# JuanTarrio/rebvo

Hardware: NVIDIA H100
Metric: frames/sec @752x480 EuRoC replay (synthetic stand-in), detect+track+map; pose ATE vs reference in `parity` (higher is better)
Workload: dtype f32 scale space/detector + f64 tracker/EKF

## Files before the change

rebvo_b200/csrc/capi.cu:

```cuda
#include <math.h>
#include <stdlib.h>
#include <new>

#include "common.cuh"
#include "tracker.cuh"

int rb_detect_upload_pinv(rb_ctx *c, const double *tab);

static void box_plan_one(double sigma, int box_n, int *box_d, double *sigma_r) {
    const double wideal = sqrt(12 * sigma * sigma / box_n + 1);
    int wl = (int)wideal;
    const int tmp = wl / 2;
    if (tmp * 2 == wl) wl--;
    const int m = (int)round((3 * box_n + 4 * box_n * wl + box_n * wl * wl - 12 * sigma * sigma) / (4 + 4 * wl));
    int i = 0;
    for (; i < m && i < box_n; i++) box_d[i] = wl;
    for (; i < box_n; i++) box_d[i] = wl + 2;
    *sigma_r = sqrt((m * wl * wl + (box_n - m) * (wl + 2.0) * (wl + 2.0) - box_n) / 12.0);
}

static void plane_fit_pinv(int ws, double *out) {
    const int n = (2 * ws + 1) * (2 * ws + 1);
    double Phi[(2 * RB_PLANE_FIT_MAX + 1) * (2 * RB_PLANE_FIT_MAX + 1)][3];
    int k = 0;
// ... 28 lines not shown
    for (int r = 0; r < 3; r++)
        for (k = 0; k < n; k++) {
            double s = 0;
            for (int c = 0; c < 3; c++) s += B[r][c] * Phi[k][c];
            out[r * n + k] = s;
        }
}

static const double *plane_fit_tables() {
    static double tab[RB_PINV_DOUBLES];
    static std::once_flag once;
    std::call_once(once, [] {
        for (int r = 1; r <= RB_PLANE_FIT_MAX; r++) plane_fit_pinv(r, tab + rb_pinv_offset(r));
    });
    return tab;
}

__device__ __forceinline__ void pack_one(const KLSoA &kl, int i, rb_keyline *dst) {
    rb_keyline k;
    k.p_inx = kl.p_inx[i];
    float2 v = kl.m_m[i];
    k.m_m[0] = v.x; k.m_m[1] = v.y;
    v = kl.u_m[i];
    k.u_m[0] = v.x; k.u_m[1] = v.y;
    k.n_m = kl.n_m[i];
    k.score = 0.f;
    v = kl.c_p[i];
    k.c_p[0] = v.x; k.c_p[1] = v.y;
    k._pad0 = 0;
    k.rho = kl.rho[i];
    k.s_rho = kl.s_rho[i];
    k.rho_nr = RB_RHO_INIT;
    k.s_rho_nr = RB_RHO_MAX;
    k.rho0 = kl.rho0[i];
    k.s_rho0 = kl.s_rho0[i];
    v = kl.p_m[i];
    k.p_m[0] = v.x; k.p_m[1] = v.y;
    v = kl.p_m_0[i];
    k.p_m_0[0] = v.x; k.p_m_0[1] = v.y;
    k.m_id = kl.m_id[i];
    k.m_id_f = kl.m_id_f[i];
    k.m_id_kf = -1;
    k.m_num = kl.m_num[i];
    v = kl.m_m0[i];
    k.m_m0[0] = v.x; k.m_m0[1] = v.y;
    k.n_m0 = kl.n_m0[i];
    k.p_id = kl.p_id[i];
    k.n_id = kl.n_id[i];
    k.net_id = -1;
    k.stereo_m_id = -1;
    k.stereo_rho = RB_RHO_INIT;
    k.stereo_s_rho = RB_RHO_MAX;
    *dst = k;
}
__global__ void k_pack_aos(KLSoA kl, const MapState *st, rb_keyline *out) {
    const int i = blockIdx.x * blockDim.x + threadIdx.x;
    if (i >= st->kn) return;
    pack_one(kl, i, out + i);
}

__global__ void __launch_bounds__(128) k_pack_aos_ind(KLSoA kl, const MapState *st, unsigned char *const *base, size_t offset) {
    __shared__ __align__(16) rb_keyline rec[128];
    const int kn = st->kn;
    const int i0 = blockIdx.x * 128;
    if (i0 >= kn) return;
    const int i = i0 + threadIdx.x;
    if (i < kn) pack_one(kl, i, &rec[threadIdx.x]);
    __syncthreads();
    const int nrec = kn - i0 < 128 ? kn - i0 : 128;
    const int n8 = nrec * (int)(sizeof(rb_keyline) / 8);
    uint2 *dst = reinterpret_cast<uint2 *>(*base + offset) + (size_t)i0 * (sizeof(rb_keyline) / 8);
    const uint2 *src = reinterpret_cast<const uint2 *>(rec);
    for (int k = threadIdx.x; k < n8; k += 128) dst[k] = src[k];
}
int rb_map_pack_aos_enqueue(rb_ctx *c, rb_map *m, unsigned char *const *base, size_t offset) {
    k_pack_aos_ind<<<rb_div_up(c->kcap, 128), 128, 0, c->stream>>>(m->kl, m->st, base, offset);
    RB_LAUNCH_CHECK();
    return RB_OK;
}

__global__ void k_unpack_aos(KLSoA kl, MapState *st, const rb_keyline *in, int kn) {
    const int i = blockIdx.x * blockDim.x + threadIdx.x;
    if (i == 0) st->kn = kn;
    if (i >= kn) return;
    const rb_keyline k = in[i];
    kl.p_inx[i] = k.p_inx;
    kl.m_m[i] = make_float2(k.m_m[0], k.m_m[1]);
    kl.u_m[i] = make_float2(k.u_m[0], k.u_m[1]);
    kl.n_m[i] = k.n_m;
    kl.c_p[i] = make_float2(k.c_p[0], k.c_p[1]);
    kl.rho[i] = k.rho;
    kl.s_rho[i] = k.s_rho;
    kl.rho0[i] = k.rho0;
    kl.s_rho0[i] = k.s_rho0;
    kl.p_m[i] = make_float2(k.p_m[0], k.p_m[1]);
    kl.p_m_0[i] = make_float2(k.p_m_0[0], k.p_m_0[1]);
    kl.m_id[i] = k.m_id;
    kl.m_id_f[i] = k.m_id_f;
    kl.m_num[i] = k.m_num;
    kl.m_m0[i] = make_float2(k.m_m0[0], k.m_m0[1]);
    kl.n_m0[i] = k.n_m0;
    kl.p_id[i] = k.p_id;
    kl.n_id[i] = k.n_id;
    kl.pack[2 * i] = make_float4(k.m_m[0], k.m_m[1], k.c_p[0], k.c_p[1]);
    kl.pack[2 * i + 1] = make_float4(k.u_m[0], k.u_m[1], k.n_m, 0.f);
}

__global__ void k_fill_int(int *p, int v, size_t n) {
    size_t i = (size_t)blockIdx.x * blockDim.x + threadIdx.x;
    if (i < n) p[i] = v;
}

extern "C" int rb_ctx_create(rb_ctx **out, int device, const rb_camera *cam, double sigma0, double ksigma,
                             int kl_capacity) {
    if (!out || !cam) return RB_ERR_ARG;
    *out = nullptr;
    int ndev = 0;
    if (cudaGetDeviceCount(&ndev) != cudaSuccess || ndev <= 0 || device >= ndev) return RB_ERR_NO_DEVICE;
    if (cam->w % 4 || cam->w < 32 || cam->h < 32 || kl_capacity < 1) return RB_ERR_ARG;
    rb_ctx *c = new (std::nothrow) rb_ctx;
    if (!c) return RB_ERR_ARG;
    memset(c, 0, sizeof(*c));
    c->mtx = new (std::nothrow) std::recursive_mutex;
    if (!c->mtx) {
        delete c;
        return RB_ERR_ARG;
    }
    c->device = device;
    c->cam = *cam;
    c->w = cam->w;
    c->h = cam->h;
    c->N = cam->w * cam->h;
    c->ppx = cam->ppx;
    c->ppy = cam->ppy;
    c->zfm = (double)((cam->zfx + cam->zfy) / 2);
    c->sigma0 = sigma0;
    c->ksigma = ksigma;
    c->kcap = kl_capacity;
    {
        const char *ds = getenv("REBVO_B200_DOG_SUB");
        c->dog_sub = ds ? atoi(ds) : 0;
        if (c->dog_sub < 0) c->dog_sub = 0;
        const char *pd = getenv("REBVO_B200_PDL");
        c->pdl = !(pd && atoi(pd) == 0);
        const char *mp = getenv("REBVO_B200_MIN_PERSIST");
        c->min_persist = !(mp && atoi(mp) == 0);
        const char *mc = getenv("REBVO_B200_MIN_CLUSTER");
        c->min_cluster = !(mc && atoi(mc) == 0);
        const char *rs = getenv("REBVO_B200_ROWSCAN");
        c->rowscan_mode = rs ? atoi(rs) : 2;
        c->mu_xchg = !(getenv("REBVO_B200_MU_XCHG") && atoi(getenv("REBVO_B200_MU_XCHG")) == 0);
        c->row_ns = getenv("REBVO_B200_ROW_NS") ? atoi(getenv("REBVO_B200_ROW_NS")) : 0;
        c->colscan_mode = getenv("REBVO_B200_COLSCAN") ? atoi(getenv("REBVO_B200_COLSCAN")) : 0;
    }
    box_plan_one(sigma0, 3, c->plan.d[0], &c->plan.sigma_r[0]);
    box_plan_one(c->plan.sigma_r[0] * ksigma, 3, c->plan.d[1], &c->plan.sigma_r[1]);
    int r = RB_OK;
    auto fail = [&](int code) {
        *out = c;
        return code;
    };
#define CK(call)                                                                                  \
    do {                                                                                          \
        cudaError_t e__ = (call);                                                                 \
        if (e__ != cudaSuccess) {                                                                 \
            snprintf(c->err, sizeof(c->err), "%s:%d %s: %s", __FILE__, __LINE__, #call,           \
                     cudaGetErrorString(e__));                                                    \
            return fail(RB_ERR_CUDA);                                                             \
        }                                                                                         \
    } while (0)
    CK(cudaSetDevice(device));
    cudaDeviceProp prop;
    CK(cudaGetDeviceProperties(&prop, device));
    c->sm_count = prop.multiProcessorCount;
    rb_minimizer_cluster_setup(c);
    if ((r = rb_dog_device_setup(c))) return fail(r);
    {
        int lo = 0, hi = 0;
        cudaDeviceGetStreamPriorityRange(&lo, &hi);
        const char *pe = getenv("REBVO_B200_PRIO");
        CK(cudaStreamCreateWithPriority(&c->stream, cudaStreamNonBlocking, (pe && atoi(pe) == 0) ? lo : hi));
    }
    c->nseg = c->h * rb_div_up(c->w, 32);
    CK(cudaMalloc(&c->seg_cnt, sizeof(int) * c->nseg));
    CK(cudaMalloc(&c->cand, sizeof(float4) * (size_t)c->N));
    c->red_cap = 1024;
    CK(cudaMalloc(&c->red_part, sizeof(double) * 32 * c->red_cap));
    CK(cudaMalloc(&c->ticket, sizeof(unsigned int) * 16));
    CK(cudaMemset(c->ticket, 0, sizeof(unsigned int) * 16));
    CK(cudaMallocHost(&c->pinned, 1 << 16));
    CK(cudaMalloc(&c->dev_small, 1 << 16));
    CK(cudaMemset(c->dev_small, 0, 1 << 16));
    {
        const int mm_init[2] = {-1, 0x7f7fffff};
        CK(cudaMemcpy((char *)c->dev_small + RB_DS_REEST, mm_init, sizeof(mm_init), cudaMemcpyHostToDevice));
    }
    if ((r = rb_detect_upload_pinv(c, plane_fit_tables()))) return fail(r);
    if ((r = rb_dog_make_tables(c))) return fail(r);
#undef CK
    *out = c;
    return RB_OK;
}

extern "C" void rb_ctx_destroy(rb_ctx *c) {
    if (!c) return;
    cudaSetDevice(c->device);
    if (c->stream) {
        cudaStreamSynchronize(c->stream);
        cudaStreamDestroy(c->stream);
    }
    cudaFree(c->seg_cnt);
    cudaFree(c->cand);
    cudaFree(c->red_part);
    cudaFree(c->ticket);
    cudaFree(c->dev_small);
    cudaFree(c->boxtab);
    if (c->pinned) cudaFreeHost(c->pinned);
    delete c->mtx;
    delete c;
}

extern "C" const char *rb_last_error(const rb_ctx *c) { return c ? c->err : "null context"; }

extern "C" int rb_ctx_sync(rb_ctx *c) {
    if (!c) return RB_ERR_ARG;
    RB_ENTER(c);
    RB_CUDA(cudaStreamSynchronize(c->stream));
    return RB_OK;
}

extern "C" int rb_ctx_box_plan(const rb_ctx *c, int *out_d, double *out_sigma_r) {
    for (int f = 0; f < 2; f++) {
        for (int i = 0; i < 3; i++) out_d[f * 3 + i] = c->plan.d[f][i];
        out_sigma_r[f] = c->plan.sigma_r[f];
    }
    return RB_OK;
}

extern "C" int64_t rb_ctx_launch_count(const rb_ctx *c) { return c->launches; }

int rb_map_alloc(rb_ctx *c, rb_map **out, bool with_ws) {
    rb_map *m = new (std::nothrow) rb_map;
    if (!m) return RB_ERR_ARG;
    memset(m, 0, sizeof(*m));
    m->c = c;
    *out = m;
    const size_t N = c->N, K = c->kcap + 32;
    RB_CUDA(cudaSetDevice(c->device));
    RB_CUDA(cudaMalloc(&m->mask, sizeof(int) * N));
    RB_CUDA(cudaMalloc(&m->field, sizeof(unsigned long long) * N));
    RB_CUDA(cudaMemsetAsync(m->field, 0xff, sizeof(unsigned long long) * N, c->stream));
    k_fill_int<<<(unsigned)((N + 255) / 256), 256, 0, c->stream>>>(m->mask, -1, N);
    RB_LAUNCH_CHECK();
    KLSoA &k = m->kl;
    RB_CUDA(cudaMalloc(&k.p_inx, sizeof(int) * K));
    RB_CUDA(cudaMalloc(&k.m_m, sizeof(float2) * K));
    RB_CUDA(cudaMalloc(&k.u_m, sizeof(float2) * K));
    RB_CUDA(cudaMalloc(&k.c_p, sizeof(float2) * K));
    RB_CUDA(cudaMalloc(&k.p_m, sizeof(float2) * K));
    RB_CUDA(cudaMalloc(&k.p_m_0, sizeof(float2) * K));
    RB_CUDA(cudaMalloc(&k.m_m0, sizeof(float2) * K));
    RB_CUDA(cudaMalloc(&k.n_m, sizeof(float) * K));
    RB_CUDA(cudaMalloc(&k.rho, sizeof(double) * K));
    RB_CUDA(cudaMalloc(&k.s_rho, sizeof(double) * K));
    RB_CUDA(cudaMalloc(&k.rho0, sizeof(double) * K));
    RB_CUDA(cudaMalloc(&k.s_rho0, sizeof(double) * K));
    RB_CUDA(cudaMalloc(&k.n_m0, sizeof(double) * K));
    RB_CUDA(cudaMalloc(&k.m_id, sizeof(int) * K));
    RB_CUDA(cudaMalloc(&k.m_id_f, sizeof(int) * K));
    RB_CUDA(cudaMalloc(&k.m_num, sizeof(int) * K));
    RB_CUDA(cudaMalloc(&k.p_id, sizeof(int) * K));
    RB_CUDA(cudaMalloc(&k.n_id, sizeof(int) * K));
    RB_CUDA(cudaMalloc(&k.pack, sizeof(float4) * 2 * K));
    RB_CUDA(cudaMalloc(&m->st, sizeof(MapState)));
    RB_CUDA(cudaMemsetAsync(m->st, 0, sizeof(MapState), c->stream));
    for (int i = 0; i < 3; i++) {
        RB_CUDA(cudaMalloc(&m->res[i], sizeof(double) * K));
        RB_CUDA(cudaMemsetAsync(m->res[i], 0, sizeof(double) * K, c->stream));
        RB_CUDA(cudaMalloc(&m->carry_flag[i], K));
        RB_CUDA(cudaMemsetAsync(m->carry_flag[i], 0, K, c->stream));
    }
    int r = rb_track_state_alloc(c, m);
    if (r) return r;
    if (with_ws) {
        if ((r = rb_dogws_alloc(c, &m->ws, 1))) return r;
        m->owns_ws = true;
        m->img0 = m->ws.img0;
        m->dog = m->ws.dog;
    }
    return RB_OK;
}

extern "C" int rb_map_create(rb_ctx *c, rb_map **out) {
    if (!c) return RB_ERR_ARG;
    RB_ENTER(c);
    if (!c || !out) return RB_ERR_ARG;
    return rb_map_alloc(c, out, true);
}

extern "C" void rb_map_destroy(rb_map *m);
extern "C" int rb_map_clone(const rb_map *src, rb_map **out) {
    if (!src) return RB_ERR_ARG;
    RB_ENTER(src->c);
    if (!src || !out) return RB_ERR_ARG;
    rb_ctx *c = src->c;
    int r = rb_map_alloc(c, out, false);
// ... 261 lines not shown
```

rebvo_b200/csrc/common.cuh:

```cuda
#pragma once
#include <cuda_runtime.h>
#include <stdint.h>
#include <stdio.h>
#include <string.h>

#include <mutex>

#include "../../include/rebvo_b200.h"

#define RB_RHO_MAX 20.0
#define RB_RHO_MIN 1e-3
#define RB_RHO_INIT 1.0
#define RB_MAX_IMG_VALUE 765

#define RB_PLANE_FIT_MAX 4
__host__ __device__ constexpr int rb_pinv_offset(int r) {
    int o = 0;
    for (int q = 1; q < r; q++) o += 3 * (2 * q + 1) * (2 * q + 1);
    return o;
}
#define RB_PINV_DOUBLES rb_pinv_offset(RB_PLANE_FIT_MAX + 1)

struct KLSoA {
    int *p_inx;
    float2 *m_m, *u_m, *c_p, *p_m, *p_m_0, *m_m0;
    float *n_m;
    double *rho, *s_rho, *rho0, *s_rho0, *n_m0;
    int *m_id, *m_id_f, *m_num, *p_id, *n_id;
    float4 *pack;
};

struct MapState {
    int kn;
    int total_cand;
    float max_dog, min_dog;
    float retuned;
    float thresh_used;
    int nmatch;
    int fwd_match;
    int reg_num;
    unsigned int frame_count;
    int do_map;
    double s_rho_q;
    double Kp, RKp;
};

struct DetChain {
    double tresh;
    int l_kl_num;
    int pad;
};

struct BoxPlan {
    int d[2][3];
    double sigma_r[2];
};

struct DogWS {
    int B;
    uint8_t *rgb;
    float *gray;
    float *S;
    float *I0;
    float *I;
    float *img0;
    float *dog;
    float *aux;
    void *tmaps;
    bool tma_ok;
    int tma_row_mask;
    bool tma_row_ok;
};

struct rb_ctx {
    std::recursive_mutex *mtx;
    int device;
    cudaStream_t stream;
    rb_camera cam;
    int w, h, N;
    float ppx, ppy;
    double zfm;
    double sigma0, ksigma;
    int kcap;
    BoxPlan plan;
    int64_t launches;
    int sm_count;
    char err[256];
    int *seg_cnt;
    int nseg;
    float4 *cand;
    double *red_part;
    int red_cap;
    unsigned int *ticket;
    void *pinned;
    void *dev_small;
    float *boxtab;
    bool counters_preset;
    int dog_sub;
    bool pdl;
    bool min_persist;
    bool min_cluster;
    int min_cluster_kpc;
    size_t min_cluster_dyn;
    int min_cluster_g;
    int min_cluster_kpc_multi;
    size_t min_cluster_dyn_multi;
    int min_debug_abort;
    bool mu_xchg;
    bool min_early;
    int min_cluster_xchg;
    int row_ns;
    int colscan_mode;
    int rowscan_mode;
};
#define RB_DS_REEST 0
#define RB_DS_CHAIN 32768
#define RB_DS_ARGS 36864
#define RB_DS_TMA_FAIL 45056
#define RB_DS_QHISTO 49152

struct LMState {
    double Xeval[6];
    int res_in, res_out;
    double max_r;
    double match_thresh, s_rho_min, k_huber;
    unsigned int match_num_thresh, frame_count;
    int iter_max, init_type, init_iter;
    double Vel_in[3], W0_in[3];
    double X[6], Xnew[6], Xt[6], h[6];
    double JtJ[36], JtF[6], JtJn[36], JtFn[6];
    double F, Fnew, F0, Ft, F0t, u, v, ut, vt, gain;
    int eff_steps, eff_steps_t;
    int iR, iRN, iRt;
    int n_eval;
    double Vel[3], W0[3], RVel[9], RW0[9], W_X[36];
    double rel_error, rel_error_score, score;
    double last_score;
    int no_keylines, pad_;
};

struct TrackState {
    LMState lm;
    int *blk_has;
    double *blk_last_fi;
    double *partials;
    double *carry;
    int nblk;
    struct MinCtl *ctl;
    unsigned long long *ll;
    struct FmBest *fm_best;
    double *reg_r, *reg_s;
    unsigned char *reg_set;
};


struct rb_map {
    rb_ctx *c;
    DogWS ws;
    bool owns_ws;
    float *img0, *dog;
    int *mask;
    unsigned long long *field;
    KLSoA kl;
    MapState *st;
    double *res[3];
    unsigned char *carry_flag[3];
    TrackState *ts;
    TrackState ts_host;
    int field_radius;
    int det_r;
};

#define RB_ENTER(ctxp)                                                \
    std::lock_guard<std::recursive_mutex> rb_lock__(*(ctxp)->mtx);    \
    cudaSetDevice((ctxp)->device)

#define RB_CUDA(call)                                                                          \
    do {                                                                                       \
        cudaError_t e__ = (call);                                                              \
        if (e__ != cudaSuccess) {                                                              \
            snprintf(c->err, sizeof(c->err), "%s:%d %s: %s", __FILE__, __LINE__, #call,        \
                     cudaGetErrorString(e__));                                                 \
            return RB_ERR_CUDA;                                                                \
        }                                                                                      \
    } while (0)

#define RB_LAUNCH_CHECK()                                                                      \
    do {                                                                                       \
        c->launches++;                                                                         \
        cudaError_t e__ = cudaGetLastError();                                                  \
        if (e__ != cudaSuccess) {                                                              \
            snprintf(c->err, sizeof(c->err), "%s:%d launch: %s", __FILE__, __LINE__,           \
                     cudaGetErrorString(e__));                                                 \
            return RB_ERR_CUDA;                                                                \
        }                                                                                      \
    } while (0)

static inline int rb_div_up(int a, int b) { return (a + b - 1) / b; }

#ifdef __CUDACC__
__device__ __forceinline__ void pdl_wait() { asm volatile("griddepcontrol.wait;" ::: "memory"); }
__device__ __forceinline__ void pdl_launch() { asm volatile("griddepcontrol.launch_dependents;" ::: "memory"); }
template <typename... KArgs, typename... Args>
static inline cudaError_t rb_klaunch(bool pdl, void (*kernel)(KArgs...), dim3 grid, dim3 block, size_t smem,
                                     cudaStream_t stream, Args... args) {
    cudaLaunchConfig_t cfg = {};
    cfg.gridDim = grid;
    cfg.blockDim = block;
    cfg.dynamicSmemBytes = smem;
    cfg.stream = stream;
    cudaLaunchAttribute attr[1];
    attr[0].id = cudaLaunchAttributeProgrammaticStreamSerialization;
    attr[0].val.programmaticStreamSerializationAllowed = 1;
    cfg.attrs = attr;
    cfg.numAttrs = pdl ? 1 : 0;
    return cudaLaunchKernelEx(&cfg, kernel, KArgs(args)...);
}
#define RB_KLAUNCH(kernel, grid, block, smem, ...)                                                  \
    do {                                                                                            \
        c->launches++;                                                                              \
        cudaError_t e__ = rb_klaunch(c->pdl, kernel, dim3(grid), dim3(block), smem, c->stream, __VA_ARGS__); \
        if (e__ != cudaSuccess) {                                                                   \
            snprintf(c->err, sizeof(c->err), "%s:%d launch: %s", __FILE__, __LINE__,                \
                     cudaGetErrorString(e__));                                                      \
            return RB_ERR_CUDA;                                                                     \
        }                                                                                           \
    } while (0)
#endif

int rb_dogws_alloc(rb_ctx *c, DogWS *ws, int B);
void rb_dogws_free(DogWS *ws);
int rb_dog_gray(rb_ctx *c, DogWS *ws, int nimg, const void *const *src_pp = nullptr);
int rb_dog_gray_mono(rb_ctx *c, DogWS *ws, int nimg, const void *const *src_pp = nullptr);
int rb_dog_build_batch(rb_ctx *c, DogWS *ws, int nimg);
int rb_dog_build_range(rb_ctx *c, DogWS *ws, int f0, int m);
int rb_dog_aux_planes(rb_ctx *c, DogWS *ws, int img);
int rb_dog_make_tables(rb_ctx *c);
int rb_dog_make_tmaps(rb_ctx *c, DogWS *ws);
int rb_dog_device_setup(rb_ctx *c);
int rb_detect_enqueue(rb_ctx *c, rb_map *m, const float *img0, const float *dog,
                      const rb_detect_params *p, DetChain *chain_dev);
int rb_reestimate_enqueue(rb_ctx *c, rb_map *m, int knum, int nbins);
```

rebvo_b200/csrc/tracker.cu:

```cuda
#include "tracker.cuh"
#include "lm.cuh"
#include "frame.cuh"

#define TVR_T 256
#define RES_SENTINEL 0x7FF8DEADBEEF0001ull

#ifdef RB_TVR_PROF
__device__ long long g_tvr_prof[256 * 16];
#define TVR_STAMP(k) do { if (threadIdx.x == 0) g_tvr_prof[blockIdx.x * 16 + (k)] = clock64(); } while (0)
__device__ __forceinline__ long long tvr_gtime() {
    long long t;
    asm volatile("mov.u64 %0, %globaltimer;" : "=l"(t));
    return t;
}
#define TVR_GSTAMP(k) do { if (threadIdx.x == 0) g_tvr_prof[blockIdx.x * 16 + (k)] = tvr_gtime(); } while (0)
extern "C" int rb_debug_fetch(long long *out) {
    return (int)cudaMemcpyFromSymbol(out, g_tvr_prof, sizeof(long long) * 256 * 16);
}
#else
#define TVR_STAMP(k) do { } while (0)
#define TVR_GSTAMP(k) do { } while (0)
#endif

struct CamC {
// ... 1219 lines not shown
    s.k_huber = k_huber;
}

int rb_try_vel_rot_enqueue(rb_ctx *c, rb_map *fmap, rb_map *old, const double *X_dev, int reweight, int procjf,
                           double match_thresh, double s_rho_min, unsigned int mnt, unsigned int fc,
                           double k_huber) {
    if (fmap->field_radius <= 0) return RB_ERR_STATE;
    k_lm_single<<<1, 1, 0, c->stream>>>(fmap->ts, X_dev, 0, 1, (double)fmap->field_radius, match_thresh, s_rho_min,
                                        mnt, fc, k_huber);
    RB_LAUNCH_CHECK();
    if (reweight && procjf) return launch_eval<true, true>(c, fmap, old, STEP_NONE);
    if (reweight) return launch_eval<true, false>(c, fmap, old, STEP_NONE);
    if (procjf) return launch_eval<false, true>(c, fmap, old, STEP_NONE);
    return launch_eval<false, false>(c, fmap, old, STEP_NONE);
}

struct RotPt {
    float2 pm;
    double rho, s_rho;
};
__device__ __forceinline__ RotPt d_rot_pt(const double (&R)[9], double zf, float2 pm, double rho, double s_rho) {
    const double v0 = (double)pm.x / zf, v1 = (double)pm.y / zf, v2 = 1;
    double q0 = 0, q1 = 0, q2 = 0;
    q0 = q0 + R[0] * v0; q0 = q0 + R[1] * v1; q0 = q0 + R[2] * v2;
    q1 = q1 + R[3] * v0; q1 = q1 + R[4] * v1; q1 = q1 + R[5] * v2;
    q2 = q2 + R[6] * v0; q2 = q2 + R[7] * v1; q2 = q2 + R[8] * v2;
    RotPt o = {pm, rho, s_rho};
    if (fabs(q2) > 0) {
        o.pm = make_float2((float)(q0 / q2 * zf), (float)(q1 / q2 * zf));
        o.rho = rho / q2;
        o.s_rho = s_rho / q2;
    }
    return o;
}
__device__ __forceinline__ float2 d_rot_m(const double (&R)[9], float2 m) {
    const double m0 = (double)m.x, m1 = (double)m.y;
    double r0 = 0, r1 = 0;
    r0 = r0 + R[0] * m0; r0 = r0 + R[1] * m1; r0 = r0 + R[2] * 0.0;
    r1 = r1 + R[3] * m0; r1 = r1 + R[4] * m1; r1 = r1 + R[5] * 0.0;
    return make_float2((float)r0, (float)r1);
}
__device__ __forceinline__ void d_rotate_vals(const KLSoA &kl, int i, const double (&R)[9], double zf, float2 pm, double rho,
                                              double s_rho, float2 m) {
    const RotPt pt = d_rot_pt(R, zf, pm, rho, s_rho);
    kl.p_m[i] = pt.pm;
    kl.rho[i] = pt.rho;
    kl.s_rho[i] = pt.s_rho;
    const float2 mr = d_rot_m(R, m);
    kl.m_m[i] = mr;
    float4 p = kl.pack[2 * i];
    p.x = mr.x;
    p.y = mr.y;
    kl.pack[2 * i] = p;
}
__device__ __forceinline__ void d_rotate(const KLSoA &kl, int i, const double *__restrict__ Rp, double zf) {
    double R[9];
#pragma unroll
    for (int k = 0; k < 9; k++) R[k] = Rp[k];
    d_rotate_vals(kl, i, R, zf, kl.p_m[i], kl.rho[i], kl.s_rho[i], kl.m_m[i]);
}
__global__ void __launch_bounds__(256) k_rotate(KLSoA kl, const MapState *st, const double *__restrict__ Rp,
                                                double zf) {
    pdl_wait();
    pdl_launch();
    const int i = blockIdx.x * blockDim.x + threadIdx.x;
    if (i >= st->kn) return;
    d_rotate(kl, i, Rp, zf);
}

__global__ void __launch_bounds__(256) k_fm_init(FmBest *best, const MapState *nst) {
    const int i = blockIdx.x * blockDim.x + threadIdx.x;
    if (i >= nst->kn) return;
    best[i] = FmBest{0ull, -1ll};
}
__global__ void __launch_bounds__(256) k_fm_argmax(KLSoA old, const MapState *ost, const MapState *nst, FmBest *best) {
    pdl_wait();
    pdl_launch();
    const int i = blockIdx.x * blockDim.x + threadIdx.x;
    if (i >= ost->kn) return;
    d_fm_argmax_one(old, i, nst->kn, best);
}
template <bool ROT>
__global__ void __launch_bounds__(256) k_fm_apply_rotate(KLSoA old, KLSoA neu, const MapState *ost, MapState *nst,
                                                         const FmBest *best, const double *__restrict__ Rp, double zf) {
    pdl_wait();
    pdl_launch();
    const int i = blockIdx.x * blockDim.x + threadIdx.x;
    const bool in = i < ost->kn;
    bool hit = false;
    double R[9], rho = 0, s_rho = 0;
#pragma unroll
    for (int k = 0; k < 9; k++) R[k] = ROT ? Rp[k] : 0.0;
    float2 pm = make_float2(0.f, 0.f), m = pm;
    if (in) {
        const int f = old.m_id_f[i];
        rho = old.rho[i];
        s_rho = old.s_rho[i];
        pm = old.p_m[i];
        m = old.m_m[i];
        if (f >= 0 && f < nst->kn && __ldcg(&best[f].idx) == i) {
            neu.rho[f] = rho;
            neu.s_rho[f] = s_rho;
            neu.m_num[f] = old.m_num[i] + 1;
            neu.m_id[f] = i;
            neu.p_m_0[f] = pm;
            neu.m_m0[f] = m;
            neu.n_m0[f] = (double)old.n_m[i];
            hit = true;
        }
    }
    const unsigned int bal = __ballot_sync(0xffffffffu, hit);
    if ((threadIdx.x & 31) == 0 && bal) atomicAdd(&nst->fwd_match, __popc(bal));
    if (ROT && in) d_rotate_vals(old, i, R, zf, pm, rho, s_rho, m);
}
__global__ void k_set_int(int *p, int v) { *p = v; }

int rb_forward_match_init_enqueue(rb_ctx *c, rb_map *neu) {
    k_fm_init<<<rb_div_up(c->kcap, 256), 256, 0, c->stream>>>(neu->ts_host.fm_best, neu->st);
    RB_LAUNCH_CHECK();
    return RB_OK;
}
int rb_forward_match_argmax_enqueue(rb_ctx *c, rb_map *old, rb_map *neu) {
    RB_KLAUNCH(k_fm_argmax, rb_div_up(c->kcap, 256), 256, 0, old->kl, (const MapState *)old->st,
               (const MapState *)neu->st, neu->ts_host.fm_best);
    return RB_OK;
}
int rb_forward_match_apply_enqueue(rb_ctx *c, rb_map *old, rb_map *neu, const double *R_dev) {
    const int nb = rb_div_up(c->kcap, 256);
    const FmBest *best = neu->ts_host.fm_best;
    if (R_dev)
        RB_KLAUNCH(k_fm_apply_rotate<true>, nb, 256, 0, old->kl, neu->kl, (const MapState *)old->st, neu->st, best, R_dev,
                   c->zfm);
    else
        RB_KLAUNCH(k_fm_apply_rotate<false>, nb, 256, 0, old->kl, neu->kl, (const MapState *)old->st, neu->st, best, R_dev,
                   c->zfm);
    return RB_OK;
}
int rb_forward_match_enqueue(rb_ctx *c, rb_map *old, rb_map *neu) {
    if (!c->counters_preset) {
        k_set_int<<<1, 1, 0, c->stream>>>(&neu->st->fwd_match, 0);
        RB_LAUNCH_CHECK();
    }
    int r;
    if ((r = rb_forward_match_init_enqueue(c, neu))) return r;
    if ((r = rb_forward_match_argmax_enqueue(c, old, neu))) return r;
    return rb_forward_match_apply_enqueue(c, old, neu, nullptr);
}

int rb_rotate_enqueue(rb_ctx *c, rb_map *m, const double *R_dev) {
    RB_KLAUNCH(k_rotate, rb_div_up(c->kcap, 256), 256, 0, m->kl, (const MapState *)m->st, R_dev, c->zfm);
    return RB_OK;
}

#define DM_G 4
template <bool ROT>
__device__ __forceinline__ int d_dm_search(const KLSoA &old, const int *__restrict__ omask,
                                           const DMatchArgs *__restrict__ ap, const CamC &cam, double min_thr_mod,
                                           double cang_min_edge, double max_radius, double loc_unc, bool valid, int g,
                                           float2 kpm, double krho, double ks_rho, float2 km, float kn_m,
                                           const double (&R)[9]) {
    const int lane = threadIdx.x & 31;
    int jm = -1;
    {
        const double zf = cam.zfm;
        const double *BR = ap->BackRot, *Vel = ap->Vel, *RV = ap->RVel;
        const double a0 = (double)kpm.x, a1 = (double)kpm.y, a2 = zf;
        double p30 = 0, p31 = 0, p32 = 0;
        p30 = p30 + BR[0] * a0; p30 = p30 + BR[1] * a1; p30 = p30 + BR[2] * a2;
        p31 = p31 + BR[3] * a0; p31 = p31 + BR[4] * a1; p31 = p31 + BR[5] * a2;
        p32 = p32 + BR[6] * a0; p32 = p32 + BR[7] * a1; p32 = p32 + BR[8] * a2;
        const float pmx = (float)(p30 * zf / p32), pmy = (float)(p31 * zf / p32);
        const double k_rho = krho * zf / p32;
        const float pi0x = pmx + cam.ppx, pi0y = pmy + cam.ppy;
        double t_x = -(Vel[0] * zf - Vel[2] * (double)pmx);
        double t_y = -(Vel[1] * zf - Vel[2] * (double)pmy);
        double norm_t = sqrt(t_x * t_x + t_y * t_y);
        const double D0 = zf, D1 = zf, D2 = (double)(-pmx - pmy);
        double r0 = 0, r1 = 0, r2 = 0;
        r0 = r0 + D0 * RV[0]; r0 = r0 + D1 * RV[3]; r0 = r0 + D2 * RV[6];
        r1 = r1 + D0 * RV[1]; r1 = r1 + D1 * RV[4]; r1 = r1 + D2 * RV[7];
        r2 = r2 + D0 * RV[2]; r2 = r2 + D1 * RV[5]; r2 = r2 + D2 * RV[8];
        double sigma2_t = 0;
        sigma2_t = sigma2_t + r0 * D0; sigma2_t = sigma2_t + r1 * D1; sigma2_t = sigma2_t + r2 * D2;
        double dq_min, dq_max, dq_rho;
        int t_steps;
        if (norm_t > 1e-6) {
            t_x /= norm_t;
            t_y /= norm_t;
            dq_rho = norm_t * k_rho;
            dq_min = fmax(0.0, norm_t * (k_rho - ks_rho)) - loc_unc;
            dq_max = fmin(max_radius, norm_t * (k_rho + ks_rho)) + loc_unc;
            if (dq_rho > dq_max) {
                dq_rho = (dq_max + dq_min) / 2;
                t_steps = (int)(dq_rho + 0.5);
            } else {
                t_steps = (int)(fmax(dq_max - dq_rho, dq_rho - dq_min) + 0.5);
            }
        } else {
            t_x = (double)km.x;
            t_y = (double)km.y;
            norm_t = (double)kn_m;
            t_x /= norm_t;
            t_y /= norm_t;
            norm_t = 1;
            dq_min = -max_radius - loc_unc;
            dq_max = max_radius + loc_unc;
            dq_rho = 0;
            t_steps = (int)dq_max;
        }
        const double norm_m = (double)kn_m;
        double tn = dq_rho, tp = dq_rho + 1;
        int t_i = g >> 1;
        const int dir = g & 1;
        for (int k = 0; k < (g >> 1); k++) {
            tp += 1;
            tn -= 1;
        }
        bool active = valid;
        while (true) {
            int j_hit = -1;
            if (active && t_i < t_steps) {
                const double t = dir ? tp : tn;
                const bool inside = dir ? !(t > dq_max) : !(t < dq_min);
                if (inside) {
                    const float fx = (float)(t_x * t + (double)pi0x), fy = (float)(t_y * t + (double)pi0y);
                    const int xi = (int)roundf(fx), yi = (int)roundf(fy);
                    if (!(xi >= cam.w || yi >= cam.h || xi < 0 || yi < 0)) {
                        const int j = omask[(size_t)yi * cam.w + xi];
                        if (j >= 0) {
                            const double norm_m0 = (double)old.n_m[j];
                            const float2 om = ROT ? d_rot_m(R, old.m_m[j]) : old.m_m[j];
                            const double cang = (double)(om.x * km.x + om.y * km.y) / (norm_m0 * norm_m);
                            if (!(cang < cang_min_edge || fabs(norm_m0 / norm_m - 1) > min_thr_mod)) {
                                double s_rho = old.s_rho[j], rho = old.rho[j];
                                if (ROT) {
                                    const RotPt pt = d_rot_pt(R, zf, old.p_m[j], rho, s_rho);
                                    rho = pt.rho;
                                    s_rho = pt.s_rho;
                                }
                                const double v_rho_dr = (loc_unc * loc_unc + s_rho * s_rho * norm_t * norm_t + sigma2_t * rho * rho);
                                const double e = t - norm_t * rho;
                                if (!(e * e > v_rho_dr)) j_hit = j;
                            }
                        }
                    }
                }
            }
            const unsigned int bal = __ballot_sync(0xffffffffu, j_hit >= 0);
            const unsigned int grp = (bal >> (lane & ~(DM_G - 1))) & ((1u << DM_G) - 1u);
            const int src = grp ? (lane & ~(DM_G - 1)) + __ffs(grp) - 1 : lane;
            const int jw = __shfl_sync(0xffffffffu, j_hit, src);
            if (grp) {
                jm = jw;
                active = false;
            }
#pragma unroll
            for (int k = 0; k < DM_G / 2; k++) {
                tp += 1;
                tn -= 1;
            }
            t_i += DM_G / 2;
            if (!__any_sync(0xffffffffu, active && t_i < t_steps)) break;
        }
    }
    return jm;
}
__global__ void __launch_bounds__(128) k_directed_match(KLSoA neu, MapState *nst, KLSoA old,
                                                        const int *__restrict__ omask, const DMatchArgs *__restrict__ ap,
                                                        CamC cam, double min_thr_mod, double cang_min_edge,
                                                        double max_radius, double loc_unc, const int *enable) {
    pdl_wait();
    pdl_launch();
    if (enable && !*enable) return;
    const int gi = blockIdx.x * blockDim.x + threadIdx.x;
    const int i = gi / DM_G, g = gi % DM_G;
    const bool valid = i < nst->kn;
    const int ic = valid ? i : 0;
    const double R[9] = {};
    int jm = d_dm_search<false>(old, omask, ap, cam, min_thr_mod, cang_min_edge, max_radius, loc_unc, valid, g,
                                neu.p_m[ic], neu.rho[ic], neu.s_rho[ic], neu.m_m[ic], neu.n_m[ic], R);
    bool got = false;
    if (g != 0) jm = -1;
    if (jm >= 0) {
        neu.rho[i] = old.rho[jm];
        neu.s_rho[i] = old.s_rho[jm];
        neu.m_id[i] = jm;
        neu.m_num[i] = old.m_num[jm] + 1;
        neu.p_m_0[i] = old.p_m[jm];
        neu.m_m0[i] = old.m_m[jm];
        neu.n_m0[i] = (double)old.n_m[jm];
        got = true;
    }
    const unsigned int bal = __ballot_sync(0xffffffffu, got);
    if ((threadIdx.x & 31) == 0 && bal) atomicAdd(&nst->nmatch, __popc(bal));
}

__global__ void __launch_bounds__(128) k_match(KLSoA neu, MapState *nst, KLSoA old, const int *__restrict__ omask,
                                               const FmBest *best, const DMatchArgs *__restrict__ ap,
                                               const double *__restrict__ Rp, double *__restrict__ reg_r,
                                               double *__restrict__ reg_s, CamC cam, double min_thr_mod,
                                               double cang_min_edge, double max_radius, double loc_unc,
                                               const int *__restrict__ do_match) {
    pdl_wait();
    pdl_launch();
    if ((int)(blockIdx.x * (blockDim.x / DM_G)) >= nst->kn) return;
    const int gi = blockIdx.x * blockDim.x + threadIdx.x;
    const int i = gi / DM_G, g = gi % DM_G;
    const bool valid = i < nst->kn;
    const int ic = valid ? i : 0;
    const longlong2 b = __ldcg(reinterpret_cast<const longlong2 *>(best + ic));
    const float2 kpm = neu.p_m[ic], km = neu.m_m[ic];
    const float kn_m = neu.n_m[ic];
    double R[9];
#pragma unroll
    for (int k = 0; k < 9; k++) R[k] = Rp[k];
    const int fw = valid ? (int)b.y : -1;
    double krho, ks_rho;
    if (fw >= 0) {
        krho = old.rho[fw];
        ks_rho = old.s_rho[fw];
    } else {
        krho = neu.rho[ic];
        ks_rho = neu.s_rho[ic];
    }
    int jm = -1;
    if (*do_match)
        jm = d_dm_search<true>(old, omask, ap, cam, min_thr_mod, cang_min_edge, max_radius, loc_unc, valid, g, kpm, krho,
                               ks_rho, km, kn_m, R);
    bool got = false;
    if (valid && g == 0) {
        double rho = krho, s_rho = ks_rho;
        if (jm >= 0) {
            const RotPt pt = d_rot_pt(R, cam.zfm, old.p_m[jm], old.rho[jm], old.s_rho[jm]);
            rho = pt.rho;
            s_rho = pt.s_rho;
            neu.m_id[i] = jm;
            neu.m_num[i] = old.m_num[jm] + 1;
            neu.p_m_0[i] = pt.pm;
            neu.m_m0[i] = d_rot_m(R, old.m_m[jm]);
            neu.n_m0[i] = (double)old.n_m[jm];
            got = true;
        } else if (fw >= 0) {
            neu.m_id[i] = fw;
            neu.m_num[i] = old.m_num[fw] + 1;
            neu.p_m_0[i] = old.p_m[fw];
            neu.m_m0[i] = old.m_m[fw];
            neu.n_m0[i] = (double)old.n_m[fw];
        }
        reg_r[i] = rho;
        reg_s[i] = s_rho;
    }
    const unsigned int bal = __ballot_sync(0xffffffffu, got);
    const unsigned int fbal = __ballot_sync(0xffffffffu, valid && g == 0 && fw >= 0);
    if ((threadIdx.x & 31) == 0) {
        if (bal) atomicAdd(&nst->nmatch, __popc(bal));
        if (fbal) atomicAdd(&nst->fwd_match, __popc(fbal));
    }
}

int rb_directed_matching_enqueue(rb_ctx *c, rb_map *neu, rb_map *old, const DMatchArgs *args_dev, double min_thr_mod,
                                 double min_thr_ang, double max_radius, double loc_uncertainty, const int *enable_dev) {
    const double cang_min_edge = cos(min_thr_ang * M_PI / 180.0);
    if (!c->counters_preset) {
        k_set_int<<<1, 1, 0, c->stream>>>(&neu->st->nmatch, 0);
        RB_LAUNCH_CHECK();
    }
    RB_KLAUNCH(k_directed_match, rb_div_up(c->kcap * DM_G, 128), 128, 0, neu->kl, neu->st, old->kl, old->mask, args_dev,
               make_cam(c), min_thr_mod, cang_min_edge, max_radius, loc_uncertainty, enable_dev);
    return RB_OK;
}
int rb_match_enqueue(rb_ctx *c, rb_map *neu, rb_map *old, const DMatchArgs *args_dev, const double *R_dev,
                     double min_thr_mod, double min_thr_ang, double max_radius, double loc_uncertainty,
                     const int *do_match_dev) {
    const double cang_min_edge = cos(min_thr_ang * M_PI / 180.0);
    const TrackState &t = neu->ts_host;
    RB_KLAUNCH(k_match, rb_div_up(c->kcap * DM_G, 128), 128, 0, neu->kl, neu->st, old->kl, (const int *)old->mask,
               (const FmBest *)t.fm_best, args_dev, R_dev, t.reg_r, t.reg_s, make_cam(c), min_thr_mod, cang_min_edge,
               max_radius, loc_uncertainty, do_match_dev);
    return RB_OK;
}

__device__ __forceinline__ bool d_reg_vals(const KLSoA &kl, int i, const double *rho, const double *s_rho, double thresh,
                                           double &r_out, double &s_out) {
    bool did = false;
    const int ni = kl.n_id[i], pi = kl.p_id[i];
    if (ni >= 0 && pi >= 0) {
        const double krho = rho[i], ks = s_rho[i];
        const double nrho = rho[ni], ns = s_rho[ni];
        const double prho = rho[pi], ps = s_rho[pi];
        const double d = nrho - prho;
        if (!(d * d > ns * ns + ps * ps)) {
            const float2 nm = kl.m_m[ni], pmv = kl.m_m[pi];
            const float nnm = kl.n_m[ni], pnm = kl.n_m[pi];
            double alpha = (double)((nm.x * pmv.x + nm.y * pmv.y) / (nnm * pnm));
            if (!(alpha - thresh < 0)) {
                alpha = (alpha - thresh) / (1 - thresh);
                alpha /= fabs(nrho - prho) / (ns + ps) + 1;
                const double wr = 1 / (ks * ks);
                const double wrn = alpha / (ns * ns);
                const double wrp = alpha / (ps * ps);
                r_out = (krho * wr + nrho * wrn + prho * wrp) / (wr + wrn + wrp);
                s_out = (ks * wr + ns * wrn + ps * wrp) / (wr + wrn + wrp);
                did = true;
            }
        }
    }
    return did;
}
__device__ __forceinline__ bool d_reg_a(const KLSoA &kl, int i, double *__restrict__ r, double *__restrict__ s,
                                        unsigned char *__restrict__ set, double thresh) {
    const bool did = d_reg_vals(kl, i, kl.rho, kl.s_rho, thresh, r[i], s[i]);
    set[i] = did ? 1 : 0;
    return did;
}
__global__ void __launch_bounds__(256) k_regularize_a(KLSoA kl, MapState *st, double *__restrict__ r,
                                                      double *__restrict__ s, unsigned char *__restrict__ set,
                                                      double thresh, const int *enable) {
    if (enable && !*enable) return;
    const int i = blockIdx.x * blockDim.x + threadIdx.x;
    const bool did = i < st->kn ? d_reg_a(kl, i, r, s, set, thresh) : false;
    const unsigned int bal = __ballot_sync(0xffffffffu, did);
    if ((threadIdx.x & 31) == 0 && bal) atomicAdd(&st->reg_num, __popc(bal));
}
__global__ void __launch_bounds__(256) k_regularize_b(KLSoA kl, const MapState *st, const double *__restrict__ r,
                                                      const double *__restrict__ s,
                                                      const unsigned char *__restrict__ set, const int *enable) {
    if (enable && !*enable) return;
    const int i = blockIdx.x * blockDim.x + threadIdx.x;
    if (i >= st->kn || !set[i]) return;
    kl.rho[i] = r[i];
    kl.s_rho[i] = s[i];
}

int rb_regularize_enqueue(rb_ctx *c, rb_map *m, double thresh, const int *enable_dev) {
    TrackState &t = m->ts_host;
    const int nb = rb_div_up(c->kcap, 256);
    if (!c->counters_preset) {
        k_set_int<<<1, 1, 0, c->stream>>>(&m->st->reg_num, 0);
        RB_LAUNCH_CHECK();
    }
    k_regularize_a<<<nb, 256, 0, c->stream>>>(m->kl, m->st, t.reg_r, t.reg_s, t.reg_set, thresh, enable_dev);
    RB_LAUNCH_CHECK();
    k_regularize_b<<<nb, 256, 0, c->stream>>>(m->kl, m->st, t.reg_r, t.reg_s, t.reg_set, enable_dev);
    RB_LAUNCH_CHECK();
    return RB_OK;
}

__device__ __forceinline__ void d_ekf(const KLSoA &kl, int i, double rho, double s_rho,
                                      const double *__restrict__ velp, double zf, double q_abs, double loc_unc) {
    const double vel0 = velp[0], vel1 = velp[1], vel2 = velp[2];
    kl.s_rho0[i] = s_rho;
    const float2 pm = kl.p_m[i], pm0 = kl.p_m_0[i], mm0 = kl.m_m0[i];
    const double n_m0 = kl.n_m0[i];
    const double qx = (double)pm.x, qy = (double)pm.y, q0x = (double)pm0.x, q0y = (double)pm0.y;
    double v_rho = s_rho * s_rho;
    const double u_x = (double)mm0.x / n_m0, u_y = (double)mm0.y / n_m0;
    const double Y = u_x * (qx - q0x) + u_y * (qy - q0y);
    const double H = u_x * (vel0 * zf - vel2 * q0x) + u_y * (vel1 * zf - vel2 * q0y);
    const double rho_p = 1 / (1.0 / rho + vel2);
    kl.rho0[i] = rho_p;
    double F = 1 / (1 + rho * vel2);
    F = F * F;
    const double p_p = F * v_rho * F + q_abs * q_abs;
    const double e = Y - H * rho_p;
    const double S = H * p_p * H + loc_unc * loc_unc;
    const double K = p_p * H * (1 / S);
    rho = rho_p + (K * e);
    v_rho = (1 - K * H) * p_p;
    s_rho = sqrt(v_rho);
    if (rho < RB_RHO_MIN) {
        s_rho += RB_RHO_MIN - rho;
        rho = RB_RHO_MIN;
    } else if (rho > RB_RHO_MAX) {
        rho = RB_RHO_MAX;
    } else if (isnan(rho) || isnan(s_rho) || isinf(rho) || isinf(s_rho)) {
        rho = RB_RHO_INIT;
        s_rho = RB_RHO_MAX;
    } else if (s_rho < 0) {
        rho = RB_RHO_INIT;
        s_rho = RB_RHO_MAX;
    }
    kl.rho[i] = rho;
    kl.s_rho[i] = s_rho;
}
__global__ void __launch_bounds__(256) k_ekf(KLSoA kl, const MapState *st, const double *__restrict__ velp, double zf,
                                             double q_abs, double loc_unc, const int *enable) {
    if (enable && !*enable) return;
    const int i = blockIdx.x * blockDim.x + threadIdx.x;
    if (i >= st->kn) return;
    if (kl.m_id[i] < 0) return;
    d_ekf(kl, i, kl.rho[i], kl.s_rho[i], velp, zf, q_abs, loc_unc);
}
int rb_ekf_enqueue(rb_ctx *c, rb_map *m, const double *vel_dev, double q_abs, double loc_unc, const int *enable_dev) {
    k_ekf<<<rb_div_up(c->kcap, 256), 256, 0, c->stream>>>(m->kl, m->st, vel_dev, c->zfm, q_abs, loc_unc, enable_dev);
    RB_LAUNCH_CHECK();
    return RB_OK;
}

__global__ void __launch_bounds__(256) k_regularize_a_gate(KLSoA kl, MapState *st, double *__restrict__ r,
                                                           double *__restrict__ s, unsigned char *__restrict__ set,
                                                           double thresh, FrameState *fs, int match_threshold) {
    pdl_wait();
    pdl_launch();
    const bool en = fs->do_match && st->nmatch >= match_threshold;
    if (blockIdx.x == 0 && threadIdx.x == 0) {
        d_frame_post_match(fs, st, match_threshold);
        st->do_map = fs->do_map;
    }
    if (!en) return;
    const int i = blockIdx.x * blockDim.x + threadIdx.x;
    const bool did = i < st->kn ? d_reg_a(kl, i, r, s, set, thresh) : false;
    const unsigned int bal = __ballot_sync(0xffffffffu, did);
    if ((threadIdx.x & 31) == 0 && bal) atomicAdd(&st->reg_num, __popc(bal));
}
__global__ void __launch_bounds__(256) k_regb_ekf(KLSoA kl, const MapState *st, const double *__restrict__ r,
                                                  const double *__restrict__ s,
                                                  const unsigned char *__restrict__ set,
                                                  const double *__restrict__ velp, double zf, double q_abs,
                                                  double loc_unc, const int *enable, FrameState *pose_fs,
                                                  const MapState *ost, const LMState *lm, rb_nav *nav,
                                                  const FrameArgs *fa) {
    pdl_wait();
    pdl_launch();
    if (pose_fs && blockIdx.x == gridDim.x - 1 && threadIdx.x == 0) {
        if (nav) d_frame_finish(pose_fs, st, ost, lm->score, nav, fa, false);
        else d_frame_pose(pose_fs);
    }
    if (enable && !*enable) return;
    const int i = blockIdx.x * blockDim.x + threadIdx.x;
// ... 380 lines not shown
```

Baseline: 7600.

## Batch directed-match line search: fewer lanes per keyline, several steps per iteration

```diff
diff --git a/rebvo_b200/csrc/capi.cu b/rebvo_b200/csrc/capi.cu
--- a/rebvo_b200/csrc/capi.cu
+++ b/rebvo_b200/csrc/capi.cu
@@ -204,6 +204,7 @@
         c->mu_xchg = !(getenv("REBVO_B200_MU_XCHG") && atoi(getenv("REBVO_B200_MU_XCHG")) == 0);
         c->row_ns = getenv("REBVO_B200_ROW_NS") ? atoi(getenv("REBVO_B200_ROW_NS")) : 0;
         c->colscan_mode = getenv("REBVO_B200_COLSCAN") ? atoi(getenv("REBVO_B200_COLSCAN")) : 0;
+        c->dm_batch = !(getenv("REBVO_B200_DM_BATCH") && atoi(getenv("REBVO_B200_DM_BATCH")) == 0);
     }
     box_plan_one(sigma0, 3, c->plan.d[0], &c->plan.sigma_r[0]);
     box_plan_one(c->plan.sigma_r[0] * ksigma, 3, c->plan.d[1], &c->plan.sigma_r[1]);
diff --git a/rebvo_b200/csrc/common.cuh b/rebvo_b200/csrc/common.cuh
--- a/rebvo_b200/csrc/common.cuh
+++ b/rebvo_b200/csrc/common.cuh
@@ -111,6 +111,7 @@
     int min_cluster_xchg;
     int row_ns;
     int colscan_mode;
+    bool dm_batch;
     int rowscan_mode;
 };
 #define RB_DS_REEST 0
diff --git a/rebvo_b200/csrc/tracker.cu b/rebvo_b200/csrc/tracker.cu
--- a/rebvo_b200/csrc/tracker.cu
+++ b/rebvo_b200/csrc/tracker.cu
@@ -1395,13 +1395,21 @@
     return RB_OK;
 }
 
-#define DM_G 4
-template <bool ROT>
+#ifndef DM_G
+#define DM_G 2
+#endif
+#ifndef DM_P
+#define DM_P 4
+#endif
+#define DM_G_SEQ 4
+template <bool ROT, int G, int P>
 __device__ __forceinline__ int d_dm_search(const KLSoA &old, const int *__restrict__ omask,
                                            const DMatchArgs *__restrict__ ap, const CamC &cam, double min_thr_mod,
                                            double cang_min_edge, double max_radius, double loc_unc, bool valid, int g,
                                            float2 kpm, double krho, double ks_rho, float2 km, float kn_m,
                                            const double (&R)[9]) {
+    static_assert(32 % G == 0 && (G == 1 || G % 2 == 0), "DM_G: 1 or an even divisor of 32");
+    static_assert(P >= 0 && (G > 1 || P % 2 == 0), "DM_P: even with one lane per keyline");
     const int lane = threadIdx.x & 31;
     int jm = -1;
     {
@@ -1460,7 +1468,96 @@
             tn -= 1;
         }
         bool active = valid;
-        while (true) {
+        if constexpr (P > 0) {
+            constexpr int PP = G > 1 ? 1 : 2;
+            constexpr int TS = G > 1 ? G / 2 : 1;
+            while (true) {
+                const double tp0 = tp, tn0 = tn;
+                int jj[P];
+#pragma unroll
+                for (int q = 0; q < P / PP; q++) {
+#pragma unroll
+                    for (int d = 0; d < PP; d++) {
+                        const int k = q * PP + d, dk = G > 1 ? dir : d;
+                        const double t = dk ? tp : tn;
+                        const bool inside = dk ? !(t > dq_max) : !(t < dq_min);
+                        jj[k] = -1;
+                        if (active && t_i + q * TS < t_steps && inside) {
+                            const float fx = (float)(t_x * t + (double)pi0x), fy = (float)(t_y * t + (double)pi0y);
+                            const int xi = (int)roundf(fx), yi = (int)roundf(fy);
+                            if (!(xi >= cam.w || yi >= cam.h || xi < 0 || yi < 0)) jj[k] = yi * cam.w + xi;
+                        }
+                    }
+#pragma unroll
+                    for (int s = 0; s < TS; s++) {
+                        tp += 1;
+                        tn -= 1;
+                    }
+                }
+#pragma unroll
+                for (int k = 0; k < P; k++) jj[k] = jj[k] >= 0 ? omask[jj[k]] : -1;
+                float nm[P];
+                float2 mm[P];
+#pragma unroll
+                for (int k = 0; k < P; k++)
+                    if (jj[k] >= 0) {
+                        nm[k] = old.n_m[jj[k]];
+                        mm[k] = old.m_m[jj[k]];
+                    }
+                int k_hit = -1;
+                double tpb = tp0, tnb = tn0;
+#pragma unroll
+                for (int q = 0; q < P / PP; q++) {
+#pragma unroll
+                    for (int d = 0; d < PP; d++) {
+                        const int k = q * PP + d, dk = G > 1 ? dir : d;
+                        const int j = jj[k];
+                        if (k_hit < 0 && j >= 0) {
+                            const double norm_m0 = (double)nm[k];
+                            const float2 om = ROT ? d_rot_m(R, mm[k]) : mm[k];
+                            const double cang = (double)(om.x * km.x + om.y * km.y) / (norm_m0 * norm_m);
+                            if (!(cang < cang_min_edge || fabs(norm_m0 / norm_m - 1) > min_thr_mod)) {
+                                double s_rho = old.s_rho[j], rho = old.rho[j];
+                                if (ROT) {
+                                    const RotPt pt = d_rot_pt(R, zf, old.p_m[j], rho, s_rho);
+                                    rho = pt.rho;
+                                    s_rho = pt.s_rho;
+                                }
+                                const double v_rho_dr = (loc_unc * loc_unc + s_rho * s_rho * norm_t * norm_t + sigma2_t * rho * rho);
+                                const double e = (dk ? tpb : tnb) - norm_t * rho;
+                                if (!(e * e > v_rho_dr)) k_hit = k;
+                            }
+                        }
+                    }
+#pragma unroll
+                    for (int s = 0; s < TS; s++) {
+                        tpb += 1;
+                        tnb -= 1;
+                    }
+                }
+                int s_hit = INT_MAX, j_hit = -1;
+#pragma unroll
+                for (int k = 0; k < P; k++)
+                    if (k == k_hit) {
+                        s_hit = 2 * (t_i + (k / PP) * TS) + (G > 1 ? dir : k % PP);
+                        j_hit = jj[k];
+                    }
+#pragma unroll
+                for (int o = 1; o < G; o <<= 1) {
+                    const int so = __shfl_xor_sync(0xffffffffu, s_hit, o), jo = __shfl_xor_sync(0xffffffffu, j_hit, o);
+                    if (so < s_hit) {
+                        s_hit = so;
+                        j_hit = jo;
+                    }
+                }
+                if (s_hit != INT_MAX) {
+                    jm = j_hit;
+                    active = false;
+                }
+                t_i += (P / PP) * TS;
+                if (!__any_sync(0xffffffffu, active && t_i < t_steps)) break;
+            }
+        } else while (true) {
             int j_hit = -1;
             if (active && t_i < t_steps) {
                 const double t = dir ? tp : tn;
@@ -1490,24 +1587,25 @@
                 }
             }
             const unsigned int bal = __ballot_sync(0xffffffffu, j_hit >= 0);
-            const unsigned int grp = (bal >> (lane & ~(DM_G - 1))) & ((1u << DM_G) - 1u);
-            const int src = grp ? (lane & ~(DM_G - 1)) + __ffs(grp) - 1 : lane;
+            const unsigned int grp = (bal >> (lane & ~(G - 1))) & ((1u << G) - 1u);
+            const int src = grp ? (lane & ~(G - 1)) + __ffs(grp) - 1 : lane;
             const int jw = __shfl_sync(0xffffffffu, j_hit, src);
             if (grp) {
                 jm = jw;
                 active = false;
             }
 #pragma unroll
-            for (int k = 0; k < DM_G / 2; k++) {
+            for (int k = 0; k < G / 2; k++) {
                 tp += 1;
                 tn -= 1;
             }
-            t_i += DM_G / 2;
+            t_i += G / 2;
             if (!__any_sync(0xffffffffu, active && t_i < t_steps)) break;
         }
     }
     return jm;
 }
+template <int G, int P>
 __global__ void __launch_bounds__(128) k_directed_match(KLSoA neu, MapState *nst, KLSoA old,
                                                         const int *__restrict__ omask, const DMatchArgs *__restrict__ ap,
                                                         CamC cam, double min_thr_mod, double cang_min_edge,
@@ -1516,12 +1614,12 @@
     pdl_launch();
     if (enable && !*enable) return;
     const int gi = blockIdx.x * blockDim.x + threadIdx.x;
-    const int i = gi / DM_G, g = gi % DM_G;
+    const int i = gi / G, g = gi % G;
     const bool valid = i < nst->kn;
     const int ic = valid ? i : 0;
     const double R[9] = {};
-    int jm = d_dm_search<false>(old, omask, ap, cam, min_thr_mod, cang_min_edge, max_radius, loc_unc, valid, g,
-                                neu.p_m[ic], neu.rho[ic], neu.s_rho[ic], neu.m_m[ic], neu.n_m[ic], R);
+    int jm = d_dm_search<false, G, P>(old, omask, ap, cam, min_thr_mod, cang_min_edge, max_radius, loc_unc, valid, g,
+                                      neu.p_m[ic], neu.rho[ic], neu.s_rho[ic], neu.m_m[ic], neu.n_m[ic], R);
     bool got = false;
     if (g != 0) jm = -1;
     if (jm >= 0) {
@@ -1538,6 +1636,7 @@
     if ((threadIdx.x & 31) == 0 && bal) atomicAdd(&nst->nmatch, __popc(bal));
 }
 
+template <int G, int P>
 __global__ void __launch_bounds__(128) k_match(KLSoA neu, MapState *nst, KLSoA old, const int *__restrict__ omask,
                                                const FmBest *best, const DMatchArgs *__restrict__ ap,
                                                const double *__restrict__ Rp, double *__restrict__ reg_r,
@@ -1546,9 +1645,9 @@
                                                const int *__restrict__ do_match) {
     pdl_wait();
     pdl_launch();
-    if ((int)(blockIdx.x * (blockDim.x / DM_G)) >= nst->kn) return;
+    if ((int)(blockIdx.x * (blockDim.x / G)) >= nst->kn) return;
     const int gi = blockIdx.x * blockDim.x + threadIdx.x;
-    const int i = gi / DM_G, g = gi % DM_G;
+    const int i = gi / G, g = gi % G;
     const bool valid = i < nst->kn;
     const int ic = valid ? i : 0;
     const longlong2 b = __ldcg(reinterpret_cast<const longlong2 *>(best + ic));
@@ -1568,8 +1667,8 @@
     }
     int jm = -1;
     if (*do_match)
-        jm = d_dm_search<true>(old, omask, ap, cam, min_thr_mod, cang_min_edge, max_radius, loc_unc, valid, g, kpm, krho,
-                               ks_rho, km, kn_m, R);
+        jm = d_dm_search<true, G, P>(old, omask, ap, cam, min_thr_mod, cang_min_edge, max_radius, loc_unc, valid, g, kpm,
+                                     krho, ks_rho, km, kn_m, R);
     bool got = false;
     if (valid && g == 0) {
         double rho = krho, s_rho = ks_rho;
@@ -1608,8 +1707,10 @@
         k_set_int<<<1, 1, 0, c->stream>>>(&neu->st->nmatch, 0);
         RB_LAUNCH_CHECK();
     }
-    RB_KLAUNCH(k_directed_match, rb_div_up(c->kcap * DM_G, 128), 128, 0, neu->kl, neu->st, old->kl, old->mask, args_dev,
-               make_cam(c), min_thr_mod, cang_min_edge, max_radius, loc_uncertainty, enable_dev);
+    auto k = c->dm_batch ? k_directed_match<DM_G, DM_P> : k_directed_match<DM_G_SEQ, 0>;
+    const int g = c->dm_batch ? DM_G : DM_G_SEQ;
+    RB_KLAUNCH(k, rb_div_up(c->kcap * g, 128), 128, 0, neu->kl, neu->st, old->kl, old->mask, args_dev, make_cam(c),
+               min_thr_mod, cang_min_edge, max_radius, loc_uncertainty, enable_dev);
     return RB_OK;
 }
 int rb_match_enqueue(rb_ctx *c, rb_map *neu, rb_map *old, const DMatchArgs *args_dev, const double *R_dev,
@@ -1617,7 +1718,9 @@
                      const int *do_match_dev) {
     const double cang_min_edge = cos(min_thr_ang * M_PI / 180.0);
     const TrackState &t = neu->ts_host;
-    RB_KLAUNCH(k_match, rb_div_up(c->kcap * DM_G, 128), 128, 0, neu->kl, neu->st, old->kl, (const int *)old->mask,
+    auto k = c->dm_batch ? k_match<DM_G, DM_P> : k_match<DM_G_SEQ, 0>;
+    const int g = c->dm_batch ? DM_G : DM_G_SEQ;
+    RB_KLAUNCH(k, rb_div_up(c->kcap * g, 128), 128, 0, neu->kl, neu->st, old->kl, (const int *)old->mask,
                (const FmBest *)t.fm_best, args_dev, R_dev, t.reg_r, t.reg_s, make_cam(c), min_thr_mod, cang_min_edge,
                max_radius, loc_uncertainty, do_match_dev);
     return RB_OK;
```

After: 7588 (median of 6 runs). No clear change (-0.2%).
